# anitasyang/Laplace-GNN

Hardware: AMD Instinct MI355X
Metric: la.fit() samples/sec (GCN, KFAC) (higher is better)
Workload: dtype f32; 1 GPU; arxiv-shaped 2-layer GCN, hessian_structure=kron (BASELINE configs[2]); num_nodes=169343, nnz=2501719, features=128, hidden=256, classes=40, n_train=90941, batch_size=10000, batches=10, parallelism=dp1 ((batch, class) units, contiguous balanced runs)

## Files before the change

### laplace-gnn_amd/csrc/paths_fused.hip

```cpp
#include "gram256.h"
#include "paths.h"

namespace lgnn {
namespace {

constexpr int kYStride = 272;
constexpr int kPlaneDwords = 512;
constexpr int kGroupDwords = 3 * kPlaneDwords;
constexpr int kYGroups = kYRows / 4;
__device__ __forceinline__ int piece_swap(int q) { return (q ^ (q >> 2)) & 1; }
__device__ __forceinline__ int piece_col(int c) { return 8 * (c >> 2) + 4 * (((c >> 1) & 1) ^ piece_swap(c >> 2)) + 2 * (c & 1); }

struct alignas(16) FusedShared {
  union {
    uint32_t pc[2][kYGroups][3][kPlaneDwords];
    float y[2][kYRows][kYStride];
  };
  int ready[4], done[4];
};
static_assert(sizeof(FusedShared) <= 160 * 1024, "the CU's LDS");

__device__ __forceinline__ int lds_min4(const int* c) {
  int4 v;
  asm volatile("ds_read_b128 %0, %1\n\ts_waitcnt lgkmcnt(0)" : "=v"(v) : "v"(uint32_t(reinterpret_cast<uintptr_t>(c))) : "memory");
  return __builtin_amdgcn_readfirstlane(min(min(v.x, v.y), min(v.z, v.w)));
}
__device__ __forceinline__ void lds_publish(int* c, int value, int lane) {
  if (lane == 0)
    asm volatile("ds_write_b32 %0, %1\n\ts_waitcnt lgkmcnt(0)" :: "v"(uint32_t(reinterpret_cast<uintptr_t>(c))), "v"(value) : "memory");
}

using i32x4 = int __attribute__((ext_vector_type(4)));
__device__ __forceinline__ i32x4 make_rsrc(const void* p, uint64_t bytes) {
  const uint64_t u = reinterpret_cast<uint64_t>(p);
  return i32x4{int(uint32_t(u)), int(uint32_t(u >> 32) & 0xffffu), int(uint32_t(bytes > 0xffffffffull ? 0xffffffffull : bytes)),
               0x00020000};
}
template <bool LIST>
struct NodeRanges {
  i32x4 prs, lrs;
  uint32_t r;
  int64_t base, cnt;
  uint32_t n0;
  __device__ __forceinline__ void init(const int32_t* __restrict__ pptr, const int32_t* __restrict__ list, int64_t n0_, int64_t N,
                                       int64_t nn, int64_t cnt_) {
    prs = make_rsrc(pptr, uint64_t(N + 1) * 4);
    lrs = make_rsrc(LIST ? list : pptr, uint64_t(LIST ? nn : 0) * 4);
    n0 = uint32_t(n0_); cnt = cnt_;
    fill(0);
  }
  __device__ __forceinline__ void fill(int64_t b) {
    base = b;
    const uint32_t ii = uint32_t(b) + (threadIdx.x & 31u);
    const bool in = int64_t(ii) < cnt;
    const uint32_t k = blockIdx.x + ii * gridDim.x;
    uint32_t node = k;
    if constexpr (LIST)
      asm volatile("buffer_load_dword %0, %1, %2, 0 offen\n\ts_waitcnt vmcnt(0)" : "=&v"(node) : "v"(in ? k * 4u : 0xfffffff0u), "s"(lrs) : "memory");
    const uint32_t off = in ? (n0 + node) * 4u + ((threadIdx.x >> 3) & 4u) : 0xfffffff0u;
    asm volatile("buffer_load_dword %0, %1, %2, 0 offen\n\ts_waitcnt vmcnt(0)" : "=&v"(r) : "v"(off), "s"(prs) : "memory");
  }
  __device__ __forceinline__ void get(int64_t i, int32_t& p0, int32_t& p1) {
    if (i - base >= 32) fill(i);
    const int l = int(i - base);
    p0 = __builtin_amdgcn_readlane(int(r), l); p1 = __builtin_amdgcn_readlane(int(r), l + 32);
  }
};

template <int OFF>
__device__ __forceinline__ void bload4(f32x4& d, uint32_t voff, const i32x4& rsrc) {
  asm volatile("buffer_load_dwordx4 %0, %1, %2, 0 offen offset:%3" : "=v"(d) : "v"(voff), "s"(rsrc), "n"(OFF) : "memory");
}
__device__ __forceinline__ void bload1(uint32_t& d, uint32_t voff, const i32x4& rsrc) {
  asm volatile("buffer_load_dword %0, %1, %2, 0 offen" : "=v"(d) : "v"(voff), "s"(rsrc) : "memory");
}
using bf16x8 = __attribute__((ext_vector_type(8))) __bf16;
using u32x4v = __attribute__((ext_vector_type(4))) uint32_t;
using u32x2v = __attribute__((ext_vector_type(2))) uint32_t;

__device__ __forceinline__ uint32_t pk_bf16(float lo, float hi) {
  using bf16x2 = __attribute__((ext_vector_type(2))) __bf16;
  const bf16x2 v = {static_cast<__bf16>(lo), static_cast<__bf16>(hi)};
  return __builtin_bit_cast(uint32_t, v);
}
__device__ __forceinline__ void split_pair(float ya, float yb, uint32_t& q0, uint32_t& q1, uint32_t& q2) {
  q0 = pk_bf16(ya, yb);
  asm("" : "+v"(q0));
  const float r1a = ya - __uint_as_float(q0 << 16), r1b = yb - __uint_as_float(q0 & 0xffff0000u);
  q1 = pk_bf16(r1a, r1b);
  asm("" : "+v"(q1));
  q2 = pk_bf16(r1a - __uint_as_float(q1 << 16), r1b - __uint_as_float(q1 & 0xffff0000u));
}

struct PTables {
  i32x4 coef, b, g, mask, pm, pv, pw;
};

struct PMeta { uint32_t oc, ob, om, w; };
__device__ __forceinline__ void meta_issue(const PTables& tb, int32_t p0, int32_t p1, int lane, PMeta& t) {
  const uint32_t q = uint32_t(max(min(p0 + lane, p1 - 1), 0)) * 4u;
  bload1(t.oc, q, tb.pm);
  bload1(t.om, q, tb.pv);
  bload1(t.w, q, tb.pw);
}
template <int YOUNGER>
__device__ __forceinline__ void meta_finish(int32_t p0, int32_t p1, int lane, uint32_t row_bytes, uint32_t mask_bytes, PMeta& t) {
  asm volatile("s_waitcnt vmcnt(%3)" : "+v"(t.oc), "+v"(t.om), "+v"(t.w) : "n"(YOUNGER) : "memory");
  const bool in = p0 + lane < p1;
  const uint32_t m = in ? t.oc : 0u, v = in ? t.om : 0u;
  t.oc = m * uint32_t(kCoefRow * 4); t.ob = m * row_bytes; t.om = v * mask_bytes;
  t.w = in ? t.w : 0u;
}

struct PLane {
  int kq;
  uint32_t oc, ob, om;
  int mshift;
};

struct POps {
  f32x4 ca[3];
  f32x4 b4, g4;
  uint32_t mw;
  float w;
};

template <bool NOBG> constexpr int kStepLoads = NOBG ? 2 : 6;
template <bool NOBG>
__device__ __forceinline__ void p_load(const PTables& tb, const PMeta& mt, int s, const PLane& pl, POps& o) {
  const int src = 4 * s + pl.kq;
  const uint32_t oc = uint32_t(__shfl(int(mt.oc), src)) + pl.oc;
  const uint32_t om = uint32_t(__shfl(int(mt.om), src)) + pl.om;
  o.w = __uint_as_float(uint32_t(__shfl(int(mt.w), src)));
  bload4<0>(o.ca[0], oc, tb.coef);
  if constexpr (!NOBG) {
    const uint32_t ob = uint32_t(__shfl(int(mt.ob), src)) + pl.ob;
    bload4<kCoefStride * 4>(o.ca[1], oc, tb.coef);
    bload4<2 * kCoefStride * 4>(o.ca[2], oc, tb.coef);
    bload4<0>(o.b4, ob, tb.b);
    bload4<0>(o.g4, ob, tb.g);
  }
  bload1(o.mw, om, tb.mask);
}
template <bool NOBG, int YOUNGER>
__device__ __forceinline__ void p_wait(POps& o) {
  if constexpr (NOBG)
    asm volatile("s_waitcnt vmcnt(%2)" : "+v"(o.ca[0]), "+v"(o.mw) : "n"(YOUNGER) : "memory");
  else
    asm volatile("s_waitcnt vmcnt(%6)" : "+v"(o.ca[0]), "+v"(o.ca[1]), "+v"(o.ca[2]), "+v"(o.b4), "+v"(o.g4), "+v"(o.mw)
                 : "n"(YOUNGER) : "memory");
}

struct PCur { float a1[3], a2[3], bb[4], gg[4]; };
struct PAlpha { u32x4v a[3], m[4]; };
constexpr uint32_t kHiHalves = 0x07060302u;
template <bool NOBG, bool HI, bool SB>
__device__ __forceinline__ void p_xform(const POps& o, const PLane& pl, PCur& c, PAlpha& al, bool bg) {
#pragma unroll
  for (int t = 0; t < 3; ++t) {
    const int tt = HI ? 3 : t;
    if (HI && t > 0) {
      if constexpr (!SB) al.a[t][0] = 0u;
      al.a[t][1] = 0u; al.a[t][2] = 0u;
      continue;
    }
    float av = o.w * o.ca[0][tt];
    asm("" : "+v"(av));
    const uint32_t h0 = __float_as_uint(av) & 0xffff0000u;
    const float r1 = av - __uint_as_float(h0);
    const float r2 = r1 - __uint_as_float(__float_as_uint(r1) & 0xffff0000u);
    if constexpr (!SB) {
      al.a[t][0] = __builtin_amdgcn_perm(__float_as_uint(r1), __float_as_uint(av), kHiHalves);
      al.a[t][1] = __float_as_uint(r2) >> 16;
    } else {
      al.a[t][1] |= h0;
      al.a[t][2] = __builtin_amdgcn_perm(__float_as_uint(r2), __float_as_uint(r1), kHiHalves);
    }
  }
  const int bits = int(o.mw >> pl.mshift);
#pragma unroll
  for (int ct = 0; ct < 4; ++ct) {
    const int on = __builtin_amdgcn_sbfe(bits, ct, 1);
    if constexpr (!SB) {
      al.m[ct][0] = uint32_t(on) & 0x3f803f80u;
      al.m[ct][1] = uint32_t(on) & 0x00003f80u;
    } else {
      al.m[ct][1] |= uint32_t(on) & 0x3f800000u;
      al.m[ct][2] = uint32_t(on) & 0x3f803f80u;
    }
  }
  if constexpr (!NOBG) {
    if (bg) {
#pragma unroll
      for (int t = 0; t < 3; ++t) {
        const int tt = HI ? 3 : t;
        c.a1[t] = (HI && t > 0) ? 0.f : o.w * o.ca[1][tt];
        c.a2[t] = (HI && t > 0) ? 0.f : o.w * o.ca[2][tt];
      }
#pragma unroll
      for (int ct = 0; ct < 4; ++ct) {
        const int on = __builtin_amdgcn_sbfe(bits, ct, 1);
        c.bb[ct] = __uint_as_float(uint32_t(on) & __float_as_uint(o.b4[ct]));
        c.gg[ct] = __uint_as_float(uint32_t(on) & __float_as_uint(o.g4[ct]));
      }
    }
  }
}
template <bool NOBG>
__device__ __forceinline__ void p_keep(const PCur& c) {
  if constexpr (!NOBG) {
    asm volatile("" :: "v"(c.a1[0]), "v"(c.a1[1]), "v"(c.a1[2]), "v"(c.a2[0]), "v"(c.a2[1]), "v"(c.a2[2]));
    asm volatile("" :: "v"(c.bb[0]), "v"(c.bb[1]), "v"(c.bb[2]), "v"(c.bb[3]), "v"(c.gg[0]), "v"(c.gg[1]), "v"(c.gg[2]), "v"(c.gg[3]));
  }
}
__device__ __forceinline__ f32x4 mfma_bf16(u32x4v a, u32x4v b, f32x4 c) {
  return __builtin_amdgcn_mfma_f32_16x16x32_bf16(__builtin_bit_cast(bf16x8, a), __builtin_bit_cast(bf16x8, b), c, 0, 0, 0);
}
__device__ __forceinline__ void p_mfma(const PCur& c, f32x4 (&y2)[3][4]) {
#pragma unroll
  for (int t = 0; t < 3; ++t)
#pragma unroll
    for (int ct = 0; ct < 4; ++ct) y2[t][ct] = __builtin_amdgcn_mfma_f32_16x16x4f32(c.a1[t], c.bb[ct], y2[t][ct], 0, 0, 0);
#pragma unroll
  for (int t = 0; t < 3; ++t)
#pragma unroll
    for (int ct = 0; ct < 4; ++ct) y2[t][ct] = __builtin_amdgcn_mfma_f32_16x16x4f32(c.a2[t], c.gg[ct], y2[t][ct], 0, 0, 0);
}
__device__ __forceinline__ void p_mfma_first(const PCur& c, f32x4 (&y2)[3][4]) {
  const f32x4 zero = {0.f, 0.f, 0.f, 0.f};
#pragma unroll
  for (int t = 0; t < 3; ++t)
#pragma unroll
    for (int ct = 0; ct < 4; ++ct) y2[t][ct] = __builtin_amdgcn_mfma_f32_16x16x4f32(c.a1[t], c.bb[ct], zero, 0, 0, 0);
#pragma unroll
  for (int t = 0; t < 3; ++t)
#pragma unroll
    for (int ct = 0; ct < 4; ++ct) y2[t][ct] = __builtin_amdgcn_mfma_f32_16x16x4f32(c.a2[t], c.gg[ct], y2[t][ct], 0, 0, 0);
}
template <bool FIRST>
__device__ __forceinline__ void p_mfma_alpha(const PAlpha& al, f32x4 (&t1)[3][4]) {
  const f32x4 zero = {0.f, 0.f, 0.f, 0.f};
#pragma unroll
  for (int t = 0; t < 3; ++t)
#pragma unroll
    for (int ct = 0; ct < 4; ++ct) t1[t][ct] = mfma_bf16(al.a[t], al.m[ct], FIRST ? zero : t1[t][ct]);
}

template <bool LIST>
struct ChunkGen {
  int64_t gi;
  int32_t gp, gend;
  int32_t pa0, pa1;
  NodeRanges<LIST> nr;
  __device__ __forceinline__ void init(const int32_t* __restrict__ pptr, const int32_t* __restrict__ list, int64_t n0, int64_t N,
                                       int64_t nn, int64_t cnt) {
    nr.init(pptr, list, n0, N, nn, cnt);
    gi = 0;
    nr.get(0, gp, gend);
    nr.get(1, pa0, pa1);
  }
  __device__ __forceinline__ void next(int64_t cnt, int32_t& q0, int32_t& q1, bool& last) {
    q0 = gp; q1 = min(gp + 64, gend);
    last = q1 >= gend;
    if (last) {
      ++gi;
      gp = pa0; gend = pa1;
      nr.get(gi + 1, pa0, pa1);
    } else {
      gp = q1;
    }
  }
};

template <bool NOBG, bool HI>
__device__ __forceinline__ void pair_body(const PTables& tb, const PMeta& mx, int sx, const PLane& pl, POps& A, POps& B, PCur& cA,
                                          PCur& cB, PAlpha& al, f32x4 (&t1)[3][4], f32x4 (&y2)[3][4], bool first, bool half) {
  constexpr int NL = kStepLoads<NOBG>;
  p_wait<NOBG, NL>(A);
  p_xform<NOBG, HI, false>(A, pl, cA, al, true);
  p_keep<NOBG>(cB);
  p_load<NOBG>(tb, mx, sx, pl, A);
  if constexpr (!NOBG) {
    if (first) p_mfma_first(cA, y2);
    else p_mfma(cA, y2);
  }
  p_wait<NOBG, NL>(B);
  p_xform<NOBG, HI, true>(B, pl, cB, al, !half);
  p_keep<NOBG>(cA);
  p_load<NOBG>(tb, mx, sx + 1, pl, B);
  if (first) p_mfma_alpha<true>(al, t1);
  else p_mfma_alpha<false>(al, t1);
  if constexpr (!NOBG)
    if (!half) p_mfma(cB, y2);
}
template <bool LIST, bool NOBG, bool HI>
__device__ __forceinline__ void product_role(const YArgs& a, const int32_t* __restrict__ pptr, const int32_t* __restrict__ list,
                                             FusedShared& sh, int64_t nn, int64_t cnt, int cg) {
  const int lane = threadIdx.x & 63;
  const int H = a.H;
  const bool path_wave = 64 * cg < H;
  if (!path_wave) return;
  PLane pl;
  const int li = lane & 15;
  pl.kq = lane >> 4;
  const int col = 64 * cg + 4 * li;
  const bool col_ok = col < H;
  pl.oc = 16u * uint32_t(li);
  pl.ob = col_ok ? 4u * uint32_t(col) : 0u;
  pl.om = col_ok ? 4u * uint32_t(col >> 5) : 0x7ffffff0u;
  pl.mshift = col & 31;
  const uint32_t row_bytes = uint32_t(H) * 4u, mask_bytes = uint32_t(a.mask_words) * 4u;
  PTables tb;
  tb.coef = make_rsrc(a.coef, uint64_t(a.n_coef) * kCoefRow * 4);
  tb.b = make_rsrc(a.bg, uint64_t(a.M) * row_bytes);
  tb.g = make_rsrc(a.bg + a.M * int64_t(H), uint64_t(a.M) * row_bytes);
  tb.mask = make_rsrc(a.mask, uint64_t(a.N) * mask_bytes);
  tb.pm = make_rsrc(a.pm, uint64_t(a.cap) * 4);
  tb.pv = make_rsrc(a.pv, uint64_t(a.cap) * 4);
  tb.pw = make_rsrc(a.pw, uint64_t(a.cap) * 4);
  const uint32_t w1_row_bytes = uint32_t(a.w1_ld) * 4u;
  const i32x4 w1rs = make_rsrc(a.W1 + int64_t(a.c0) * a.w1_ld, uint64_t(a.R - 1) * w1_row_bytes + row_bytes);
  constexpr int NL = kStepLoads<NOBG>;
  ChunkGen<LIST> gen;
  gen.init(pptr, list, a.n0, a.N, nn, cnt);
  int32_t q0c, q1c, q0n, q1n;
  bool lastc, lastn;
  gen.next(cnt, q0c, q1c, lastc);
  gen.next(cnt, q0n, q1n, lastn);
  PMeta mc, mn;
  meta_issue(tb, q0c, q1c, lane, mc);
  meta_issue(tb, q0n, q1n, lane, mn);
  meta_finish<0>(q0c, q1c, lane, row_bytes, mask_bytes, mc);
  meta_finish<0>(q0n, q1n, lane, row_bytes, mask_bytes, mn);
  POps A, B;
  p_load<NOBG>(tb, mc, 0, pl, A);
  p_load<NOBG>(tb, mc, 1, pl, B);
  f32x4 t1[3][4], y2[3][4];
#pragma unroll
  for (int t = 0; t < 3; ++t)
#pragma unroll
    for (int ct = 0; ct < 4; ++ct) { t1[t][ct] = f32x4{0.f, 0.f, 0.f, 0.f}; y2[t][ct] = f32x4{0.f, 0.f, 0.f, 0.f}; }
  PCur cA = {}, cB = {};
  PAlpha al;
#pragma unroll
  for (int t = 0; t < 3; ++t) al.a[t] = u32x4v{0u, 0u, 0u, 0u};
#pragma unroll
  for (int ct = 0; ct < 4; ++ct) al.m[ct] = u32x4v{0u, 0u, 0u, 0u};
  bool node_has = false;
  bool firstc = true;
  for (int64_t i = 0; i < cnt;) {
    int32_t q0f, q1f;
    bool lastf;
    gen.next(cnt, q0f, q1f, lastf);
    PMeta mf2;
    meta_issue(tb, q0f, q1f, lane, mf2);
    const int kch = q1c - q0c, np = max((kch + 7) >> 3, 1);
    node_has = node_has || kch > 0;
#pragma clang loop unroll(disable)
    for (int j = 0; j < np; ++j) {
      const bool more = j + 1 < np;
      PMeta mx;
      mx.oc = more ? mc.oc : mn.oc; mx.ob = more ? mc.ob : mn.ob; mx.om = more ? mc.om : mn.om; mx.w = more ? mc.w : mn.w;
      const int sx = more ? 2 * (j + 1) : 0;
      const bool first = firstc && j == 0, half = !more && 4 * (2 * j + 1) >= kch;
      pair_body<NOBG, HI>(tb, mx, sx, pl, A, B, cA, cB, al, t1, y2, first, half);
    }
    if (lastc) {
      int wl = lane;
      asm volatile("" : "+v"(wl));
      const int wkq = wl >> 4, wcol = 64 * cg + 4 * (wl & 15);
      const bool wcol_ok = wcol < H;
      const uint32_t w1_off = wcol_ok ? uint32_t(4 * wkq) * w1_row_bytes + 4u * uint32_t(wcol) : 0x7ff00000u;
      const int pc_lo = 8 * (wcol >> 2) + 4 * piece_swap(wcol >> 2), pc_hi = pc_lo ^ 4;
      f32x4 w1[3][4];
#pragma unroll
      for (int t = 0; t < 3; ++t)
#pragma unroll
        for (int r = 0; r < 4; ++r) bload4<0>(w1[t][r], w1_off + uint32_t(16 * t + r) * w1_row_bytes, w1rs);
      if (i >= 2)
        while (lds_min4(sh.done) < int(i) - 1) __builtin_amdgcn_s_sleep(2);
#pragma unroll
      for (int t = 0; t < 3; ++t)
        asm volatile("s_waitcnt vmcnt(0)" : "+v"(w1[t][0]), "+v"(w1[t][1]), "+v"(w1[t][2]), "+v"(w1[t][3]) :: "memory");
      asm volatile("s_nop 11" ::: "memory");
      __builtin_amdgcn_sched_barrier(0);
      if (node_has && wcol_ok) {
        if (a.gram_f32) {
          float (*ytile)[kYStride] = sh.y[i & 1];
#pragma unroll
          for (int t = 0; t < 3; ++t)
#pragma unroll
            for (int r = 0; r < 4; ++r) {
              f32x4 o;
#pragma unroll
              for (int ct = 0; ct < 4; ++ct) o[ct] = w1[t][r][ct] * t1[t][ct][r] + y2[t][ct][r];
              *reinterpret_cast<f32x4*>(&ytile[16 * t + 4 * wkq + r][wcol]) = o;
            }
        } else {
          uint32_t* __restrict__ grp = &sh.pc[i & 1][wkq][0][0];
#pragma unroll
          for (int t = 0; t < 3; ++t) {
            u32x4v pz[3][2];
#pragma unroll
            for (int ct = 0; ct < 4; ++ct)
#pragma unroll
              for (int rp = 0; rp < 2; ++rp) {
                const float ya = w1[t][2 * rp][ct] * t1[t][ct][2 * rp] + y2[t][ct][2 * rp];
                const float yb = w1[t][2 * rp + 1][ct] * t1[t][ct][2 * rp + 1] + y2[t][ct][2 * rp + 1];
                uint32_t q0, q1, q2;
                split_pair(ya, yb, q0, q1, q2);
                pz[0][ct >> 1][2 * (ct & 1) + rp] = q0;
                pz[1][ct >> 1][2 * (ct & 1) + rp] = q1;
                pz[2][ct >> 1][2 * (ct & 1) + rp] = q2;
              }
            uint32_t* __restrict__ g = grp + 4 * t * kGroupDwords;
            *reinterpret_cast<u32x4v*>(g + pc_lo) = pz[2][0];
            *reinterpret_cast<u32x4v*>(g + pc_hi) = pz[2][1];
            *reinterpret_cast<u32x4v*>(g + kPlaneDwords + pc_lo) = pz[0][0];
            *reinterpret_cast<u32x4v*>(g + kPlaneDwords + pc_hi) = pz[0][1];
            *reinterpret_cast<u32x4v*>(g + 2 * kPlaneDwords + pc_lo) = pz[1][0];
            *reinterpret_cast<u32x4v*>(g + 2 * kPlaneDwords + pc_hi) = pz[1][1];
          }
        }
      }
      ++i;
      lds_publish(&sh.ready[cg], int(i), lane);
#pragma unroll
      for (int t = 0; t < 3; ++t) {
        asm volatile("" : "=v"(t1[t][0]), "=v"(t1[t][1]), "=v"(t1[t][2]), "=v"(t1[t][3]));
        if constexpr (!NOBG) asm volatile("" : "=v"(y2[t][0]), "=v"(y2[t][1]), "=v"(y2[t][2]), "=v"(y2[t][3]));
      }
      node_has = false;
    }
    meta_finish<2 * NL>(q0f, q1f, lane, row_bytes, mask_bytes, mf2);
    firstc = lastc;
    q0c = q0n; q1c = q1n; lastc = lastn; mc = mn;
    q0n = q0f; q1n = q1f; lastn = lastf; mn = mf2;
  }
  asm volatile("s_waitcnt vmcnt(0)" ::: "memory");
}

template <int W>
__device__ __forceinline__ void gram16_load(const float* __restrict__ p, float (&x)[8][2]) {
#pragma unroll
  for (int b = 0; b < 8; ++b) {
    x[b][0] = tiles256_uses<W>(b) ? p[b * 32] : 0.f;
    x[b][1] = tiles256_uses<W>(b) ? p[b * 32 + 16] : 0.f;
  }
}
template <int W>
__device__ __forceinline__ void gram16_mfma(const float (&x)[8][2], f32x4 (&acc)[9][2][2]) {
#pragma unroll
  for (int s = 0; s < 9; ++s)
#pragma unroll
    for (int hi = 0; hi < 2; ++hi)
#pragma unroll
      for (int hj = 0; hj < 2; ++hj) {
        if (Tiles256<W>::si[s] == Tiles256<W>::sj[s] && hi > hj) continue;
        acc[s][hi][hj] = __builtin_amdgcn_mfma_f32_16x16x4f32(x[Tiles256<W>::si[s]][hi], x[Tiles256<W>::sj[s]][hj],
                                                              acc[s][hi][hj], 0, 0, 0);
      }
}
template <int W, bool LIST>
__device__ __forceinline__ void gram_role(const YArgs& a, const int32_t* __restrict__ pptr, const int32_t* __restrict__ list,
                                          FusedShared& sh, int64_t nn, int64_t cnt, float* __restrict__ scratch) {
  const int lane = threadIdx.x & 63;
  f32x4 acc[9][2][2];
#pragma unroll
  for (int s = 0; s < 9; ++s)
#pragma unroll
    for (int q = 0; q < 4; ++q) acc[s][q >> 1][q & 1] = f32x4{0.f, 0.f, 0.f, 0.f};
  const int nk = (a.R + 3) >> 2;
  NodeRanges<LIST> nr;
  nr.init(pptr, list, a.n0, a.N, nn, cnt);
  int32_t p0, p1;
  nr.get(0, p0, p1);
  for (int64_t i = 0; i < cnt; ++i) {
    int32_t q0, q1;
    nr.get(i + 1, q0, q1);
    while (lds_min4(sh.ready) < int(i) + 1) __builtin_amdgcn_s_sleep(2);
    if (p1 > p0) {
      const float* __restrict__ base = &sh.y[i & 1][0][0] + (lane >> 4) * kYStride + (lane & 15);
      float xa[8][2], xb[8][2];
      gram16_load<W>(base, xa);
      for (int kk = 0; kk < nk; kk += 2) {
        if (kk + 1 < nk) gram16_load<W>(base + (kk + 1) * 4 * kYStride, xb);
        __builtin_amdgcn_sched_barrier(0);
        gram16_mfma<W>(xa, acc);
        __builtin_amdgcn_sched_barrier(0);
        if (kk + 1 < nk) {
          if (kk + 2 < nk) gram16_load<W>(base + (kk + 2) * 4 * kYStride, xa);
          __builtin_amdgcn_sched_barrier(0);
          gram16_mfma<W>(xb, acc);
          __builtin_amdgcn_sched_barrier(0);
        }
      }
    }
    lds_publish(&sh.done[W], int(i) + 1, lane);
    p0 = q0; p1 = q1;
  }
  const int64_t D = a.H;
  const int li = lane & 15, lq = lane >> 4;
#pragma unroll
  for (int s = 0; s < 9; ++s)
#pragma unroll
    for (int hi = 0; hi < 2; ++hi)
#pragma unroll
      for (int hj = 0; hj < 2; ++hj) {
        if (Tiles256<W>::si[s] == Tiles256<W>::sj[s] && hi > hj) continue;
        const int64_t jj = Tiles256<W>::sj[s] * 32 + 16 * hj + li;
#pragma unroll
        for (int r = 0; r < 4; ++r) {
          const int64_t ii = Tiles256<W>::si[s] * 32 + 16 * hi + 4 * lq + r;
          if (ii < D && jj < D) atomicAdd(&scratch[ii * D + jj], acc[s][hi][hj][r]);
        }
      }
}

struct PieceBlk { u32x4v t; u32x2v y1; };

template <int W> struct GramOrder;
template <> struct GramOrder<0> { static constexpr int o[9] = {0, 3, 4, 7, 8, 1, 2, 5, 6}; };
template <> struct GramOrder<1> { static constexpr int o[9] = {7, 8, 3, 4, 5, 6, 0, 1, 2}; };
template <> struct GramOrder<2> { static constexpr int o[9] = {7, 8, 3, 4, 5, 6, 0, 1, 2}; };
template <> struct GramOrder<3> { static constexpr int o[9] = {0, 7, 3, 5, 1, 8, 4, 6, 2}; };
template <int W> __device__ __forceinline__ constexpr int gram_last_use(int b) {
  int last = -1;
  for (int p = 0; p < 9; ++p)
    if (Tiles256<W>::si[GramOrder<W>::o[p]] == b || Tiles256<W>::sj[GramOrder<W>::o[p]] == b) last = p;
  return last;
}
template <int W> __device__ __forceinline__ constexpr int gram_first_use(int b) {
  for (int p = 0; p < 9; ++p)
    if (Tiles256<W>::si[GramOrder<W>::o[p]] == b || Tiles256<W>::sj[GramOrder<W>::o[p]] == b) return p;
  return -1;
}

__device__ __forceinline__ void piece_load(const uint32_t* __restrict__ tile, int off, int b, PieceBlk (&x)[8][2]) {
  const uint32_t* __restrict__ pe = tile + off;
  const uint32_t* __restrict__ po = tile + (off ^ 4) + 32;
  const u32x2v e2 = *reinterpret_cast<const u32x2v*>(pe + b * 64), e0 = *reinterpret_cast<const u32x2v*>(pe + kPlaneDwords + b * 64);
  const u32x2v o2 = *reinterpret_cast<const u32x2v*>(po + b * 64), o0 = *reinterpret_cast<const u32x2v*>(po + kPlaneDwords + b * 64);
  x[b][0].t = u32x4v{e2[0], e2[1], e0[0], e0[1]};
  x[b][0].y1 = *reinterpret_cast<const u32x2v*>(pe + 2 * kPlaneDwords + b * 64);
  x[b][1].t = u32x4v{o2[0], o2[1], o0[0], o0[1]};
  x[b][1].y1 = *reinterpret_cast<const u32x2v*>(po + 2 * kPlaneDwords + b * 64);
}
__device__ __forceinline__ u32x4v piece_u(const PieceBlk& p) { return u32x4v{p.t[2], p.t[3], p.y1[0], p.y1[1]}; }
__device__ __forceinline__ u32x4v piece_t(const PieceBlk& p) { return p.t; }
template <int W>
__device__ __forceinline__ void piece_chunk16(PieceBlk (&x)[8][2], f32x4 (&acc)[9][2][2], const uint32_t* __restrict__ tile, int off) {
#pragma unroll
  for (int p = 0; p < 9; ++p) {
    const int s = GramOrder<W>::o[p], si = Tiles256<W>::si[s], sj = Tiles256<W>::sj[s];
#pragma unroll
    for (int b = 0; b < 8; ++b)
      if (gram_first_use<W>(b) == p)
#pragma unroll
        for (int h = 0; h < 2; ++h) asm volatile("" : "+v"(x[b][h].t), "+v"(x[b][h].y1));
    const u32x4v ua[2] = {piece_u(x[si][0]), piece_u(x[si][1])}, ta[2] = {piece_t(x[si][0]), piece_t(x[si][1])};
    const u32x4v ub[2] = {piece_u(x[sj][0]), piece_u(x[sj][1])}, tb[2] = {piece_t(x[sj][0]), piece_t(x[sj][1])};
#pragma unroll
    for (int f = 0; f < 3; ++f)
#pragma unroll
      for (int hi = 0; hi < 2; ++hi)
#pragma unroll
        for (int hj = 0; hj < 2; ++hj) {
          if (si == sj && hi > hj) continue;
          acc[s][hi][hj] = mfma_bf16(f == 1 ? ta[hi] : ua[hi], f == 2 ? tb[hj] : ub[hj], acc[s][hi][hj]);
        }
    __builtin_amdgcn_sched_barrier(0);
#pragma unroll
    for (int b = 0; b < 8; ++b)
      if (gram_last_use<W>(b) == p) piece_load(tile, off, b, x);
  }
}
template <int W>
__device__ __forceinline__ void piece_chunk8(const PieceBlk (&x)[8][2], f32x4 (&acc)[9][2][2], bool low) {
#pragma unroll
  for (int p = 0; p < 9; ++p) {
    const int s = GramOrder<W>::o[p], si = Tiles256<W>::si[s], sj = Tiles256<W>::sj[s];
    u32x4v a1[2], a2[2];
#pragma unroll
    for (int hi = 0; hi < 2; ++hi) {
      const u32x4v u = piece_u(x[si][hi]), t = piece_t(x[si][hi]);
#pragma unroll
      for (int j = 0; j < 4; ++j) { a1[hi][j] = low ? u[j] : t[j]; a2[hi][j] = low ? u[j] : 0u; }
    }
    const u32x4v ub[2] = {piece_u(x[sj][0]), piece_u(x[sj][1])}, tb[2] = {piece_t(x[sj][0]), piece_t(x[sj][1])};
#pragma unroll
    for (int f = 0; f < 2; ++f)
#pragma unroll
      for (int hi = 0; hi < 2; ++hi)
#pragma unroll
        for (int hj = 0; hj < 2; ++hj) {
          if (si == sj && hi > hj) continue;
          acc[s][hi][hj] = mfma_bf16(f == 0 ? a1[hi] : a2[hi], f == 0 ? ub[hj] : tb[hj], acc[s][hi][hj]);
        }
    __builtin_amdgcn_sched_barrier(0);
  }
}
template <int W, bool LIST>
__device__ __forceinline__ void gram_split16_role(const YArgs& a, const int32_t* __restrict__ pptr, const int32_t* __restrict__ list,
                                                  FusedShared& sh, int64_t nn, int64_t cnt, float* __restrict__ scratch) {
  const int lane = threadIdx.x & 63;
  f32x4 acc[9][2][2];
#pragma unroll
  for (int s = 0; s < 9; ++s)
#pragma unroll
    for (int q = 0; q < 4; ++q) acc[s][q >> 1][q & 1] = f32x4{0.f, 0.f, 0.f, 0.f};
  const int n8 = (a.R + 7) >> 3, n16 = n8 >> 1;
  const bool odd = n8 & 1;
  const int gq = lane >> 4;
  const int start = (n16 > 0 ? gq : gq & 1) * kGroupDwords + piece_col(lane & 15);
  const int to_odd = (4 - 2 * (gq >> 1)) * kGroupDwords;
  NodeRanges<LIST> nr;
  nr.init(pptr, list, a.n0, a.N, nn, cnt);
  int32_t p0, p1;
  nr.get(0, p0, p1);
  for (int64_t i = 0; i < cnt; ++i) {
    int32_t q0, q1;
    nr.get(i + 1, q0, q1);
    while (lds_min4(sh.ready) < int(i) + 1) __builtin_amdgcn_s_sleep(2);
    if (p1 > p0) {
      const uint32_t* __restrict__ tile = &sh.pc[i & 1][0][0][0];
      int off = start;
      PieceBlk x[8][2];
#pragma unroll
      for (int b = 0; b < 8; ++b)
        if (tiles256_uses<W>(b)) piece_load(tile, off, b, x);
      __builtin_amdgcn_sched_barrier(0);
      for (int cc = 0; cc < n16; ++cc) {
        off += cc + 1 < n16 ? 4 * kGroupDwords : odd ? to_odd : 0;
        piece_chunk16<W>(x, acc, tile, off);
      }
      if (odd) piece_chunk8<W>(x, acc, gq < 2);
    }
    lds_publish(&sh.done[W], int(i) + 1, lane);
    p0 = q0; p1 = q1;
  }
  const int64_t D = a.H;
  const int fl = int(__builtin_amdgcn_mbcnt_hi(~0u, __builtin_amdgcn_mbcnt_lo(~0u, 0u)));
  const int li = fl & 15, lq = (fl >> 4) & 3;
#pragma unroll
  for (int s = 0; s < 9; ++s)
#pragma unroll
    for (int hi = 0; hi < 2; ++hi)
#pragma unroll
      for (int hj = 0; hj < 2; ++hj) {
        if (Tiles256<W>::si[s] == Tiles256<W>::sj[s] && hi > hj) continue;
        const int64_t jj = Tiles256<W>::sj[s] * 32 + 16 * hj + li;
#pragma unroll
        for (int r = 0; r < 4; ++r) {
          const int64_t ii = Tiles256<W>::si[s] * 32 + 16 * hi + 4 * lq + r;
          if (ii < D && jj < D && (Tiles256<W>::si[s] != Tiles256<W>::sj[s] || ii <= jj)) atomicAdd(&scratch[ii * D + jj], acc[s][hi][hj][r]);
        }
      }
}

template <bool LIST>
__global__ __launch_bounds__(512, 2) void paths_fused_kernel(YArgs a, const int32_t* __restrict__ pptr,
                                                             const int32_t* __restrict__ list, float* __restrict__ scratch) {
  __shared__ FusedShared sh;
  if (int64_t(pptr[a.N]) > a.cap) return;
  for (int q = threadIdx.x; q < int(sizeof(sh.pc) / 16); q += 512) reinterpret_cast<u32x4v*>(&sh.pc[0][0][0][0])[q] = u32x4v{0u, 0u, 0u, 0u};
  if (threadIdx.x < 4) {
    sh.ready[threadIdx.x] = 64 * int(threadIdx.x) < a.H ? 0 : INT32_MAX;
    sh.done[threadIdx.x] = 0;
  }
  __syncthreads();
  const int hw = __builtin_amdgcn_readfirstlane(int(threadIdx.x >> 6));
  const int64_t stride = gridDim.x;
  const int64_t nn = LIST ? int64_t(__builtin_amdgcn_readfirstlane(*a.n_list)) : a.n1 - a.n0;
  const int64_t cnt = nn > int64_t(blockIdx.x) ? (nn - blockIdx.x + stride - 1) / stride : 0;
  switch (hw) {
    case 4: if (a.gram_f32) gram_role<0, LIST>(a, pptr, list, sh, nn, cnt, scratch); else gram_split16_role<0, LIST>(a, pptr, list, sh, nn, cnt, scratch); break;
    case 5: if (a.gram_f32) gram_role<1, LIST>(a, pptr, list, sh, nn, cnt, scratch); else gram_split16_role<1, LIST>(a, pptr, list, sh, nn, cnt, scratch); break;
    case 6: if (a.gram_f32) gram_role<2, LIST>(a, pptr, list, sh, nn, cnt, scratch); else gram_split16_role<2, LIST>(a, pptr, list, sh, nn, cnt, scratch); break;
    case 7: if (a.gram_f32) gram_role<3, LIST>(a, pptr, list, sh, nn, cnt, scratch); else gram_split16_role<3, LIST>(a, pptr, list, sh, nn, cnt, scratch); break;
    default:
      if (a.c0 != a.cb) {
        if (a.no_bg) product_role<LIST, true, true>(a, pptr, list, sh, nn, cnt, hw);
        else product_role<LIST, false, true>(a, pptr, list, sh, nn, cnt, hw);
      } else {
        if (a.no_bg) product_role<LIST, true, false>(a, pptr, list, sh, nn, cnt, hw);
        else product_role<LIST, false, false>(a, pptr, list, sh, nn, cnt, hw);
      }
      break;
  }
}

constexpr int64_t kFusedWorkgroups = 256;

}

int launch_paths_fused(lgnn_ctx* h, YArgs y, int64_t cb, int64_t ce, float* scratch, hipStream_t s) {
  LGNN_REQUIRE(y.N < (int64_t(1) << 31), "too many nodes for one launch");
  const dim3 grid{unsigned(std::min<int64_t>(y.n1 - y.n0, kFusedWorkgroups))};
  const char* e = getenv("LGNN_GRAM_F32");
  y.Y = nullptr; y.gram_f32 = e && atoi(e) != 0 ? 1 : 0;
  for (int64_t c0 = cb; c0 < ce; c0 += kYRows) {
    y.c0 = int(c0); y.R = int(std::min<int64_t>(kYRows, ce - c0));
    if (h->timing) LGNN_CALL(record_event(h, s));
    if (y.list) hipLaunchKernelGGL(paths_fused_kernel<true>, grid, dim3(512), 0, s, y, y.pptr, y.list, scratch);
    else hipLaunchKernelGGL(paths_fused_kernel<false>, grid, dim3(512), 0, s, y, y.pptr, y.list, scratch);
    LGNN_HIP_CHECK(hipGetLastError());
    if (h->timing) { LGNN_CALL(record_event(h, s)); h->ev_planes += y.R; }
  }
  return 0;
}

}
```

Before: 2.544 million samples/s.

## Restructure split-bf16 gram piece loads to read full u/t vectors from LDS

Instead of loading a t vector plus a y1 half and rebuilding the u operand in registers, the gram split16 role now reads both t and u operands directly from LDS using byte offsets. The odd trailing 8-row chunk reads its A operand from offsets computed up front, with a small zeroed LDS region standing in for the missing plane. The intent is to drop the register shuffles and selects that feed the MFMAs and to prefetch the odd-chunk operands during the last 16-row chunk. In exchange it issues more LDS reads, uses more registers per piece, and adds 4 KB of zeroed shared memory.

```diff
diff --git a/laplace-gnn_amd/csrc/paths_fused.hip b/laplace-gnn_amd/csrc/paths_fused.hip
--- a/laplace-gnn_amd/csrc/paths_fused.hip
+++ b/laplace-gnn_amd/csrc/paths_fused.hip
@@ -8,6 +8,7 @@
 constexpr int kPlaneDwords = 512;
 constexpr int kGroupDwords = 3 * kPlaneDwords;
 constexpr int kYGroups = kYRows / 4;
+constexpr int kPlaneBytes = 4 * kPlaneDwords, kGroupBytes = 4 * kGroupDwords, kTileBytes = kYGroups * kGroupBytes;
 __device__ __forceinline__ int piece_swap(int q) { return (q ^ (q >> 2)) & 1; }
 __device__ __forceinline__ int piece_col(int c) { return 8 * (c >> 2) + 4 * (((c >> 1) & 1) ^ piece_swap(c >> 2)) + 2 * (c & 1); }
 
@@ -16,6 +17,7 @@
     uint32_t pc[2][kYGroups][3][kPlaneDwords];
     float y[2][kYRows][kYStride];
   };
+  uint32_t zero[2 * kPlaneDwords];
   int ready[4], done[4];
 };
 static_assert(sizeof(FusedShared) <= 160 * 1024, "the CU's LDS");
@@ -517,7 +519,7 @@
       }
 }
 
-struct PieceBlk { u32x4v t; u32x2v y1; };
+struct PieceBlk { u32x4v t, u; };
 
 template <int W> struct GramOrder;
 template <> struct GramOrder<0> { static constexpr int o[9] = {0, 3, 4, 7, 8, 1, 2, 5, 6}; };
@@ -530,64 +532,75 @@
     if (Tiles256<W>::si[GramOrder<W>::o[p]] == b || Tiles256<W>::sj[GramOrder<W>::o[p]] == b) last = p;
   return last;
 }
-template <int W> __device__ __forceinline__ constexpr int gram_first_use(int b) {
+template <int W> __device__ __forceinline__ constexpr int gram_first_a(int b) {
   for (int p = 0; p < 9; ++p)
-    if (Tiles256<W>::si[GramOrder<W>::o[p]] == b || Tiles256<W>::sj[GramOrder<W>::o[p]] == b) return p;
+    if (Tiles256<W>::si[GramOrder<W>::o[p]] == b) return p;
   return -1;
 }
 
-__device__ __forceinline__ void piece_load(const uint32_t* __restrict__ tile, int off, int b, PieceBlk (&x)[8][2]) {
-  const uint32_t* __restrict__ pe = tile + off;
-  const uint32_t* __restrict__ po = tile + (off ^ 4) + 32;
-  const u32x2v e2 = *reinterpret_cast<const u32x2v*>(pe + b * 64), e0 = *reinterpret_cast<const u32x2v*>(pe + kPlaneDwords + b * 64);
-  const u32x2v o2 = *reinterpret_cast<const u32x2v*>(po + b * 64), o0 = *reinterpret_cast<const u32x2v*>(po + kPlaneDwords + b * 64);
-  x[b][0].t = u32x4v{e2[0], e2[1], e0[0], e0[1]};
-  x[b][0].y1 = *reinterpret_cast<const u32x2v*>(pe + 2 * kPlaneDwords + b * 64);
-  x[b][1].t = u32x4v{o2[0], o2[1], o0[0], o0[1]};
-  x[b][1].y1 = *reinterpret_cast<const u32x2v*>(po + 2 * kPlaneDwords + b * 64);
-}
-__device__ __forceinline__ u32x4v piece_u(const PieceBlk& p) { return u32x4v{p.t[2], p.t[3], p.y1[0], p.y1[1]}; }
-__device__ __forceinline__ u32x4v piece_t(const PieceBlk& p) { return p.t; }
+__device__ __forceinline__ u32x4v piece_read(const char* __restrict__ pcs, uint32_t off) {
+  const u32x2v lo = *reinterpret_cast<const u32x2v*>(pcs + off), hi = *reinterpret_cast<const u32x2v*>(pcs + off + kPlaneBytes);
+  return u32x4v{lo[0], lo[1], hi[0], hi[1]};
+}
+__device__ __forceinline__ uint32_t piece_at(uint32_t off, int b, int h) { return (h ? (off ^ 16u) + 128u : off) + 256u * uint32_t(b); }
+__device__ __forceinline__ void piece_load(const char* __restrict__ pcs, uint32_t offt, uint32_t offu, int b, PieceBlk (&x)[8][2]) {
+#pragma unroll
+  for (int h = 0; h < 2; ++h) {
+    x[b][h].t = piece_read(pcs, piece_at(offt, b, h));
+    x[b][h].u = piece_read(pcs, piece_at(offu, b, h));
+  }
+}
+struct OddOffsets { uint32_t t, u, a; };
+__device__ __forceinline__ OddOffsets odd_offsets(uint32_t lrow, uint32_t at, uint32_t zero_at) {
+  asm volatile("" : "+v"(lrow));
+  const bool low = lrow < 2u * kGroupBytes;
+  OddOffsets o;
+  o.u = lrow + (low ? at : at - 2u * kGroupBytes);
+  o.t = low ? o.u - kPlaneBytes : zero_at + (lrow & 127u);
+  o.a = low ? o.u : o.u - kPlaneBytes;
+  return o;
+}
 template <int W>
-__device__ __forceinline__ void piece_chunk16(PieceBlk (&x)[8][2], f32x4 (&acc)[9][2][2], const uint32_t* __restrict__ tile, int off) {
+__device__ __forceinline__ void piece_load_a(const char* __restrict__ pcs, uint32_t offa, u32x4v (&xa)[8][2]) {
+#pragma unroll
+  for (int b = 0; b < 8; ++b)
+    if (gram_first_a<W>(b) == 0 || gram_first_a<W>(b) == 1) {
+#pragma unroll
+      for (int h = 0; h < 2; ++h) xa[b][h] = piece_read(pcs, piece_at(offa, b, h));
+      __builtin_amdgcn_sched_barrier(0);
+    }
+}
+template <int W, bool LAST>
+__device__ __forceinline__ void piece_chunk16(PieceBlk (&x)[8][2], u32x4v (&xa)[8][2], f32x4 (&acc)[9][2][2], const char* __restrict__ pcs,
+                                              uint32_t offt, uint32_t offu, uint32_t offa) {
 #pragma unroll
   for (int p = 0; p < 9; ++p) {
     const int s = GramOrder<W>::o[p], si = Tiles256<W>::si[s], sj = Tiles256<W>::sj[s];
 #pragma unroll
-    for (int b = 0; b < 8; ++b)
-      if (gram_first_use<W>(b) == p)
-#pragma unroll
-        for (int h = 0; h < 2; ++h) asm volatile("" : "+v"(x[b][h].t), "+v"(x[b][h].y1));
-    const u32x4v ua[2] = {piece_u(x[si][0]), piece_u(x[si][1])}, ta[2] = {piece_t(x[si][0]), piece_t(x[si][1])};
-    const u32x4v ub[2] = {piece_u(x[sj][0]), piece_u(x[sj][1])}, tb[2] = {piece_t(x[sj][0]), piece_t(x[sj][1])};
-#pragma unroll
     for (int f = 0; f < 3; ++f)
 #pragma unroll
       for (int hi = 0; hi < 2; ++hi)
 #pragma unroll
         for (int hj = 0; hj < 2; ++hj) {
           if (si == sj && hi > hj) continue;
-          acc[s][hi][hj] = mfma_bf16(f == 1 ? ta[hi] : ua[hi], f == 2 ? tb[hj] : ub[hj], acc[s][hi][hj]);
+          acc[s][hi][hj] = mfma_bf16(f == 1 ? x[si][hi].t : x[si][hi].u, f == 2 ? x[sj][hj].t : x[sj][hj].u, acc[s][hi][hj]);
         }
     __builtin_amdgcn_sched_barrier(0);
 #pragma unroll
     for (int b = 0; b < 8; ++b)
-      if (gram_last_use<W>(b) == p) piece_load(tile, off, b, x);
+      if (gram_last_use<W>(b) == p) {
+        piece_load(pcs, offt, offu, b, x);
+        __builtin_amdgcn_sched_barrier(0);
+      }
+    if (LAST && p == 7) piece_load_a<W>(pcs, offa, xa);
   }
 }
 template <int W>
-__device__ __forceinline__ void piece_chunk8(const PieceBlk (&x)[8][2], f32x4 (&acc)[9][2][2], bool low) {
+__device__ __forceinline__ void piece_chunk8(const PieceBlk (&x)[8][2], u32x4v (&xa)[8][2], f32x4 (&acc)[9][2][2],
+                                             const char* __restrict__ pcs, uint32_t offa) {
 #pragma unroll
   for (int p = 0; p < 9; ++p) {
     const int s = GramOrder<W>::o[p], si = Tiles256<W>::si[s], sj = Tiles256<W>::sj[s];
-    u32x4v a1[2], a2[2];
-#pragma unroll
-    for (int hi = 0; hi < 2; ++hi) {
-      const u32x4v u = piece_u(x[si][hi]), t = piece_t(x[si][hi]);
-#pragma unroll
-      for (int j = 0; j < 4; ++j) { a1[hi][j] = low ? u[j] : t[j]; a2[hi][j] = low ? u[j] : 0u; }
-    }
-    const u32x4v ub[2] = {piece_u(x[sj][0]), piece_u(x[sj][1])}, tb[2] = {piece_t(x[sj][0]), piece_t(x[sj][1])};
 #pragma unroll
     for (int f = 0; f < 2; ++f)
 #pragma unroll
@@ -595,9 +608,14 @@
 #pragma unroll
         for (int hj = 0; hj < 2; ++hj) {
           if (si == sj && hi > hj) continue;
-          acc[s][hi][hj] = mfma_bf16(f == 0 ? a1[hi] : a2[hi], f == 0 ? ub[hj] : tb[hj], acc[s][hi][hj]);
+          acc[s][hi][hj] = mfma_bf16(xa[si][hi], f == 0 ? x[sj][hj].u : x[sj][hj].t, acc[s][hi][hj]);
         }
     __builtin_amdgcn_sched_barrier(0);
+#pragma unroll
+    for (int b = 0; b < 8; ++b)
+      if (gram_first_a<W>(b) == p + 2)
+#pragma unroll
+        for (int h = 0; h < 2; ++h) xa[b][h] = piece_read(pcs, piece_at(offa, b, h));
   }
 }
 template <int W, bool LIST>
@@ -611,9 +629,10 @@
     for (int q = 0; q < 4; ++q) acc[s][q >> 1][q & 1] = f32x4{0.f, 0.f, 0.f, 0.f};
   const int n8 = (a.R + 7) >> 3, n16 = n8 >> 1;
   const bool odd = n8 & 1;
-  const int gq = lane >> 4;
-  const int start = (n16 > 0 ? gq : gq & 1) * kGroupDwords + piece_col(lane & 15);
-  const int to_odd = (4 - 2 * (gq >> 1)) * kGroupDwords;
+  const char* __restrict__ pcs = reinterpret_cast<const char*>(&sh.pc[0][0][0][0]);
+  const uint32_t lrow = uint32_t(lane >> 4) * kGroupBytes + 4u * uint32_t(piece_col(lane & 15));
+  const uint32_t zero_at = uint32_t(reinterpret_cast<const char*>(&sh.zero[0]) - pcs);
+  const uint32_t odd_rows = uint32_t(min(4 * n16, kYGroups - 2)) * kGroupBytes;
   NodeRanges<LIST> nr;
   nr.init(pptr, list, a.n0, a.N, nn, cnt);
   int32_t p0, p1;
@@ -623,18 +642,34 @@
     nr.get(i + 1, q0, q1);
     while (lds_min4(sh.ready) < int(i) + 1) __builtin_amdgcn_s_sleep(2);
     if (p1 > p0) {
-      const uint32_t* __restrict__ tile = &sh.pc[i & 1][0][0][0];
-      int off = start;
+      const uint32_t tile = uint32_t(i & 1) * kTileBytes;
+      const uint32_t odd_at = tile + odd_rows + kPlaneBytes;
+      uint32_t offt, offu;
+      if (n16 > 0) {
+        uint32_t r = lrow;
+        asm volatile("" : "+v"(r));
+        offt = r + tile; offu = offt + kPlaneBytes;
+      } else {
+        const OddOffsets o = odd_offsets(lrow, odd_at, zero_at);
+        offt = o.t; offu = o.u;
+      }
+      asm volatile("" : "+v"(offu));
       PieceBlk x[8][2];
+      u32x4v xa[8][2];
 #pragma unroll
       for (int b = 0; b < 8; ++b)
-        if (tiles256_uses<W>(b)) piece_load(tile, off, b, x);
-      __builtin_amdgcn_sched_barrier(0);
-      for (int cc = 0; cc < n16; ++cc) {
-        off += cc + 1 < n16 ? 4 * kGroupDwords : odd ? to_odd : 0;
-        piece_chunk16<W>(x, acc, tile, off);
-      }
-      if (odd) piece_chunk8<W>(x, acc, gq < 2);
+        if (tiles256_uses<W>(b)) {
+          piece_load(pcs, offt, offu, b, x);
+          __builtin_amdgcn_sched_barrier(0);
+        }
+      for (int cc = 0; cc + 1 < n16; ++cc) {
+        offt += 4 * kGroupBytes; offu += 4 * kGroupBytes;
+        piece_chunk16<W, false>(x, xa, acc, pcs, offt, offu, 0u);
+      }
+      const OddOffsets o = odd_offsets(lrow, odd_at, zero_at);
+      if (n16 > 0) piece_chunk16<W, true>(x, xa, acc, pcs, o.t, o.u, o.a);
+      else piece_load_a<W>(pcs, o.a, xa);
+      if (odd) piece_chunk8<W>(x, xa, acc, pcs, o.a);
     }
     lds_publish(&sh.done[W], int(i) + 1, lane);
     p0 = q0; p1 = q1;
@@ -664,6 +699,7 @@
   __shared__ FusedShared sh;
   if (int64_t(pptr[a.N]) > a.cap) return;
   for (int q = threadIdx.x; q < int(sizeof(sh.pc) / 16); q += 512) reinterpret_cast<u32x4v*>(&sh.pc[0][0][0][0])[q] = u32x4v{0u, 0u, 0u, 0u};
+  for (int q = threadIdx.x; q < int(sizeof(sh.zero) / 16); q += 512) reinterpret_cast<u32x4v*>(&sh.zero[0])[q] = u32x4v{0u, 0u, 0u, 0u};
   if (threadIdx.x < 4) {
     sh.ready[threadIdx.x] = 64 * int(threadIdx.x) < a.H ? 0 : INT32_MAX;
     sh.done[threadIdx.x] = 0;
```

Result: no change. 2.522 million samples/s, median of 2 (-0.9%).
